# jianwen-xie/Latent-Space-Normalizing-Flow

Measured on AMD Instinct MI355X. Metric: latent-samples/sec through flow+logdet, nz=128 B=65536, higher is better.
Workload: dtype bf16x3; 1 GPU; CIFAR-10 flow prior nz=128 f_width=64 f_depth=5 affine, forward+logdet+log-prob, B=65536 synthetic z per evaluation (BASELINE.json configs[2]); rows_per_gpu=65536, global_rows=65536, parallelism=single GPU, streams=3, clock_ramp_launches_before_warmup=600

## Files before the change

### latent-space-normalizing-flow_amd/csrc/lsnf_device.h

```cpp
#pragma once
#include <hip/hip_runtime.h>
#include <type_traits>
#include "lsnf_layout.h"

typedef float f32x16 __attribute__((ext_vector_type(16)));
typedef float f32x4 __attribute__((ext_vector_type(4)));

#define LSNF_WG_THREADS 256
#define LSNF_WG_WAVES 4
#define LSNF_WG_SAMPLES (LSNF_WG_WAVES * 32)

#define LSNF_AS1 __attribute__((address_space(1)))
#define LSNF_AS3 __attribute__((address_space(3)))

static inline hipError_t lsnf_allow_big_lds(const void* kernel, unsigned long long* done_mask) {
    int dev = 0;
    hipError_t e = hipGetDevice(&dev);
    if (e != hipSuccess) return e;
    if (dev >= 0 && dev < 64 && ((*done_mask >> dev) & 1ull)) return hipSuccess;
    e = hipFuncSetAttribute(kernel, hipFuncAttributeMaxDynamicSharedMemorySize, 160 * 1024);
    if (e != hipSuccess) return e;
    if (dev >= 0 && dev < 64) *done_mask |= 1ull << dev;
    return hipSuccess;
}

template <template <int, int> class Cfg, class F>
static inline auto lsnf_with_cfg(const LsnfGeo& g, F&& f) {
    if (g.HT == 1) return f(Cfg<1, 1>{});
    if (g.WT == 2) return f(Cfg<2, 2>{});
    return f(Cfg<2, 4>{});
}

static inline unsigned long long* lsnf_stamps_buffer() {
#ifdef LSNF_STAMPS
    extern unsigned long long* g_lsnf_stamps;
    if (!g_lsnf_stamps && hipMalloc(&g_lsnf_stamps, sizeof(unsigned long long) * 64 * 4 * 4096) != hipSuccess) g_lsnf_stamps = nullptr;
    return g_lsnf_stamps;
#else
    return nullptr;
#endif
}

template <int HT_, int WT_>
struct LsnfStackCfg {
    static constexpr int HT = HT_, WT = WT_, NZT = 2 * HT_;
    static constexpr int P1 = NZT, P2 = WT, P3 = WT, P4 = 2 * HT, NP = P1 + P2 + P3 + P4;
    static constexpr int KT1 = NZT, KT2 = HT, KT3 = WT, KT4 = WT;
    static constexpr int OFF_S2 = LSNF_FRAG_FLOATS * P1 * KT1;
    static constexpr int OFF_S3 = OFF_S2 + LSNF_FRAG_FLOATS * P2 * KT2;
    static constexpr int OFF_S4 = OFF_S3 + LSNF_FRAG_FLOATS * P3 * KT3;
    static constexpr int FWD_BLOCK = OFF_S4 + LSNF_FRAG_FLOATS * P4 * KT4;
    static constexpr int FWD_CONST = 32 * NP + 32;
    static constexpr int INV_BLOCK = LSNF_FRAG_FLOATS * NZT * NZT;
    static constexpr int INV_CONST = 32 * NZT;
    static constexpr int OFF_B4 = 0;
    static constexpr int OFF_B3 = OFF_B4 + LSNF_FRAG_FLOATS * WT * 2 * HT;
    static constexpr int OFF_B2 = OFF_B3 + LSNF_FRAG_FLOATS * WT * WT;
    static constexpr int OFF_B1 = OFF_B2 + LSNF_FRAG_FLOATS * HT * WT;
    static constexpr int BWD_BLOCK = OFF_B1 + LSNF_FRAG_FLOATS * NZT * NZT;
    static constexpr int MAXKT = (NZT > WT ? NZT : WT);
    static constexpr int SLOT = 2 * MAXKT * LSNF_FRAG_FLOATS;
};

#define LSNF_STATS_SLOTS 64
__device__ __forceinline__ void lsnf_publish_stats(double* stats, double sum_ll, double sum_logdet, int rows, int lane) {
    const unsigned grid = gridDim.x, wg = blockIdx.x;
    unsigned long long* ticket = reinterpret_cast<unsigned long long*>(&stats[2]);
    int last = 0;
    if (lane == 0) {
        const unsigned s = wg % LSNF_STATS_SLOTS;
        double* sub = stats + 8 + 4 * s;
        const double r0 = atomicAdd(&sub[0], sum_ll);
        const double r1 = atomicAdd(&sub[1], sum_logdet);
        unsigned long long inc = 1ull;
        asm volatile("" : "+v"(inc) : "v"(r0), "v"(r1));
        bool slot_done = true;
        if (grid > LSNF_STATS_SLOTS) {
            const unsigned long long n_s = (grid - s + LSNF_STATS_SLOTS - 1) / LSNF_STATS_SLOTS;
            unsigned long long* st = reinterpret_cast<unsigned long long*>(&sub[2]);
            slot_done = atomicAdd(st, inc) == n_s - 1;
            if (slot_done) atomicExch(st, 0ull);
            inc = 1ull;
        }
        if (slot_done) {
            const unsigned long long slots = grid > LSNF_STATS_SLOTS ? LSNF_STATS_SLOTS : grid;
            if (atomicAdd(ticket, inc) == slots - 1) { last = 1; atomicExch(ticket, 0ull); }
        }
    }
    if (__builtin_amdgcn_readfirstlane(last)) {
        unsigned long long* sub = reinterpret_cast<unsigned long long*>(stats + 8 + 4 * lane);
        double fl = __longlong_as_double((long long)atomicExch(&sub[0], 0ull));
        double fd = __longlong_as_double((long long)atomicExch(&sub[1], 0ull));
#pragma unroll
        for (int o = 32; o > 0; o >>= 1) { fl += __shfl_xor(fl, o, 64); fd += __shfl_xor(fd, o, 64); }
        if (lane == 0) { stats[4] = fl; stats[5] = fd; stats[6] = (double)rows; }
    }
}

__device__ __forceinline__ constexpr int lsnf_feat(int r, int h) { return (r & 3) + 8 * (r >> 2) + 4 * h; }

template <int KT, int NW = LSNF_WG_WAVES>
__device__ __forceinline__ void lsnf_issue_panel(const float* __restrict__ gsrc, float* lbuf, int wave, int lane) {
#ifdef LSNF_ABLATE_DMA
    return;
#endif
    constexpr int PIECES = 4 * KT;
    constexpr int PER_WAVE = (PIECES + NW - 1) / NW;
#pragma unroll
    for (int s = 0; s < PER_WAVE; ++s) {
        const int seg = s * NW + wave;
        if (PIECES % NW == 0 || seg < PIECES) {
            const float* g = gsrc + seg * 256 + lane * 4;
            float* l = lbuf + seg * 256;
            __builtin_amdgcn_global_load_lds((const LSNF_AS1 void*)g, (LSNF_AS3 void*)l, 16, 0, 0);
        }
    }
}

__device__ __forceinline__ void lsnf_panel_barrier() {
    asm volatile("s_waitcnt vmcnt(0)" ::: "memory");
#ifndef LSNF_ABLATE_BARRIER
    __syncthreads();
#endif
}

template <int KT>
__device__ __forceinline__ void lsnf_panel_mma(f32x16& acc, const f32x16* in, const float* lbuf, int lane) {
    const f32x4* wp = reinterpret_cast<const f32x4*>(lbuf) + lane;
    __builtin_amdgcn_sched_barrier(0);
    f32x4 w0 = wp[0], w1 = wp[64], w2 = wp[128], w3 = wp[192];
    __builtin_amdgcn_sched_group_barrier(0x100, 4, 0);
#pragma unroll
    for (int kt = 0; kt < KT; ++kt) {
        f32x4 n0 = w0, n1 = w1, n2 = w2, n3 = w3;
        if (kt + 1 < KT) {
            n0 = wp[((kt + 1) * 4 + 0) * 64]; n1 = wp[((kt + 1) * 4 + 1) * 64];
            n2 = wp[((kt + 1) * 4 + 2) * 64]; n3 = wp[((kt + 1) * 4 + 3) * 64];
        }
#define LSNF_MFMA4(W, G)                                                                      \
        acc = __builtin_amdgcn_mfma_f32_32x32x2f32(W[0], in[kt][4 * G + 0], acc, 0, 0, 0);    \
        acc = __builtin_amdgcn_mfma_f32_32x32x2f32(W[1], in[kt][4 * G + 1], acc, 0, 0, 0);    \
        acc = __builtin_amdgcn_mfma_f32_32x32x2f32(W[2], in[kt][4 * G + 2], acc, 0, 0, 0);    \
        acc = __builtin_amdgcn_mfma_f32_32x32x2f32(W[3], in[kt][4 * G + 3], acc, 0, 0, 0);
        LSNF_MFMA4(w0, 0) LSNF_MFMA4(w1, 1) LSNF_MFMA4(w2, 2) LSNF_MFMA4(w3, 3)
#undef LSNF_MFMA4
        if (kt + 1 < KT) __builtin_amdgcn_sched_group_barrier(0x100, 4, 0);
        __builtin_amdgcn_sched_group_barrier(0x008, 16, 0);
        w0 = n0; w1 = n1; w2 = n2; w3 = n3;
    }
}

__device__ __forceinline__ f32x16 lsnf_bias_init(const float* cst, int h) {
    const f32x4* b = reinterpret_cast<const f32x4*>(cst + h * 16);
    f32x16 a;
#pragma unroll
    for (int q = 0; q < 4; ++q) {
        const f32x4 v = b[q];
        a[4 * q + 0] = v[0]; a[4 * q + 1] = v[1]; a[4 * q + 2] = v[2]; a[4 * q + 3] = v[3];
    }
    return a;
}

__device__ __forceinline__ f32x16 lsnf_zero16() {
    f32x16 a;
#pragma unroll
    for (int r = 0; r < 16; ++r) a[r] = 0.0f;
    return a;
}

__device__ __forceinline__ f32x16 lsnf_relu16(f32x16 a) {
#pragma unroll
    for (int r = 0; r < 16; ++r) a[r] = fmaxf(a[r], 0.0f);
    return a;
}

__device__ __forceinline__ void lsnf_sigmoid_log2(float p, float& sig, float& l2) {
    const float pc = __builtin_amdgcn_fmed3f(p, -80.0f, 80.0f);
    const float e = __builtin_amdgcn_exp2f(pc * -1.4426950408889634f);
    const float d = 1.0f + e;
    sig = __builtin_amdgcn_rcpf(d);
    l2 = __builtin_amdgcn_logf(d);
}

__device__ __forceinline__ void lsnf_sigmoid_logsig(float p, float& sig, float& lsig) {
#ifdef LSNF_ABLATE_EPILOGUE
    sig = p * 0.25f + 0.5f; lsig = p; return;
#endif
#ifdef LSNF_OCML_MATH
    const float a = fabsf(p);
    const float e = expf(-a);
    const float r = 1.0f / (1.0f + e);
    const float l = log1pf(e);
    sig = (p >= 0.0f) ? r : e * r;
    lsig = fminf(p, 0.0f) - l;
#else
    float l2;
    lsnf_sigmoid_log2(p, sig, l2);
    lsig = -0.6931471805599453f * l2;
#endif
}

__device__ __forceinline__ float lsnf_pair_add16(float v) {
    const unsigned u = __builtin_bit_cast(unsigned, v);
    const auto r = __builtin_amdgcn_permlane16_swap(u, u, false, false);
    return __builtin_bit_cast(float, (unsigned)r[0]) + __builtin_bit_cast(float, (unsigned)r[1]);
}
__device__ __forceinline__ float lsnf_pair_add32(float v) {
    const unsigned u = __builtin_bit_cast(unsigned, v);
    const auto r = __builtin_amdgcn_permlane32_swap(u, u, false, false);
    return __builtin_bit_cast(float, (unsigned)r[0]) + __builtin_bit_cast(float, (unsigned)r[1]);
}
__device__ __forceinline__ unsigned lsnf_pair_or32(unsigned u) {
    const auto r = __builtin_amdgcn_permlane32_swap(u, u, false, false);
    return (unsigned)r[0] | (unsigned)r[1];
}
__device__ __forceinline__ float lsnf_pair_sum(float v) { return lsnf_pair_add32(v); }

typedef float f32x2 __attribute__((ext_vector_type(2)));
template <int HT>
__device__ __forceinline__ f32x16 lsnf_load_tile(int t, const float* __restrict__ zr, int half, int h, int vw) {
    f32x16 x;
    const int hh = t / HT, tt = t % HT;
#pragma unroll
    for (int g = 0; g < 4; ++g) {
        const int f0 = 32 * tt + 8 * g + 4 * h;
        const int col0 = hh * half + f0;
        if (vw == 4) {
            f32x4 v = {0.f, 0.f, 0.f, 0.f};
            if (f0 < half) v = *reinterpret_cast<const f32x4*>(zr + col0);
            x[4 * g + 0] = v[0]; x[4 * g + 1] = v[1]; x[4 * g + 2] = v[2]; x[4 * g + 3] = v[3];
        } else if (vw == 2) {
            f32x2 v0 = {0.f, 0.f}, v1 = {0.f, 0.f};
            if (f0 < half) v0 = *reinterpret_cast<const f32x2*>(zr + col0);
            if (f0 + 2 < half) v1 = *reinterpret_cast<const f32x2*>(zr + col0 + 2);
            x[4 * g + 0] = v0[0]; x[4 * g + 1] = v0[1]; x[4 * g + 2] = v1[0]; x[4 * g + 3] = v1[1];
        } else {
#pragma unroll
            for (int j = 0; j < 4; ++j) x[4 * g + j] = (f0 + j < half) ? zr[col0 + j] : 0.0f;
        }
    }
    return x;
}

template <int HT>
__device__ __forceinline__ void lsnf_store_tile(int t, const f32x16& x, float* __restrict__ zr, int half, int h, int vw) {
    const int hh = t / HT, tt = t % HT;
#pragma unroll
    for (int g = 0; g < 4; ++g) {
        const int f0 = 32 * tt + 8 * g + 4 * h;
// ... 189 lines not shown
```

### latent-space-normalizing-flow_amd/csrc/lsnf_fwd3p.hip

```cpp
#include <stdlib.h>
#include <type_traits>
#include "lsnf_l16.h"

#if LSNF_L16_PARTS != 3
#error "lsnf_fwd3p.hip is the three-term bf16 kernel"
#endif

#ifndef LSNF_FILLMASK
#define LSNF_FILLMASK 0x7f
#endif

namespace {

struct Fwd3pArgs {
    const float* consts; const float* panels3;
    const float* z_in; const float* objective;
    float* z_out; float* logdet_out; float* ll_out;
    int B, nz, half, n_blocks, vec4;
    double* stats;
    float* hdump; int width;
    float* z_saved; float* act_saved;
    unsigned long long* stamps;
};

// ... 118 lines not shown
    for (int r = r0; r < r0 + 2 * ST; ++r) {
        float sig, l2;
        lsnf_sigmoid_log2(p.q[qr][r], sig, l2);
        p.q[qr][r] = sig; lsum[st] += l2;
    }
    keep(p.q[qr][r0], p.q[qr][r0 + 1], p.q[qr][r0 + 2 * ST - 2], p.q[qr][r0 + 2 * ST - 1], lsum[st]);
}
template <int ST>
__device__ __forceinline__ void couple_q16(Tile16& v, const Tile16& t, const Tile16& sig, int q) {
    const int qr = unit_quad<ST>(q), r0 = 2 * unit_pair0<ST>(q);
#pragma unroll
    for (int r = r0; r < r0 + 2 * ST; ++r) v.q[qr][r] = (v.q[qr][r] + t.q[qr][r]) * sig.q[qr][r];
}

#ifndef LSNF_STASH_AUX
#define LSNF_STASH_AUX 0
#endif
#ifndef LSNF_STASH_PARTS
#define LSNF_STASH_PARTS 7
#endif
typedef unsigned u32x4s __attribute__((ext_vector_type(4)));
struct StashLane { unsigned zoff, soff, moff, msh, hoff; };
struct StashRsrc { __amdgpu_buffer_rsrc_t r[2]; };
__device__ __forceinline__ StashRsrc stash_rsrc(const float* p, unsigned bytes, unsigned second_off) {
    char* c = reinterpret_cast<char*>(const_cast<float*>(p));
    return StashRsrc{{__builtin_amdgcn_make_buffer_rsrc(c, 0, (int)bytes, 0x00020000),
                      __builtin_amdgcn_make_buffer_rsrc(c + second_off, 0, (int)(bytes > second_off ? bytes - second_off : 0u), 0x00020000)}};
}
template <int HT>
__device__ __forceinline__ void stash_row_quad(const StashRsrc& rs, const StashLane& sl, int t, int q, const Tile16& x, int nz, int half, int g) {
    if constexpr (!(LSNF_STASH_PARTS & 4)) return;
    const int ft = q >> 1, st = q & 1, hh = t / HT, tt = t % HT;
    unsigned off = sl.zoff;
    if (st) off += (unsigned)(16 * nz * 4);
    off = (32 * tt + 16 * ft + 4 * g < half) ? off : 0x80000000u;
    const u32x4s v = __builtin_bit_cast(u32x4s, x.q[q]);
    __builtin_amdgcn_raw_buffer_store_b128(v, rs.r[hh], off + (unsigned)((32 * tt + 16 * ft) * 4), 0, LSNF_STASH_AUX);
}
__device__ __forceinline__ void stash_sigma_quad(const StashRsrc& rs, const StashLane& sl, int t, int q, const Tile16& sg) {
    if constexpr (!(LSNF_STASH_PARTS & 2)) return;
    const int ft = q >> 1, st = q & 1;
    const u32x4s v = __builtin_bit_cast(u32x4s, sg.q[q]);
    __builtin_amdgcn_raw_buffer_store_b128(v, rs.r[t], sl.soff + (unsigned)((2 * ft * 64 + 16 * st) * 16), 0, LSNF_STASH_AUX);
}
__device__ __forceinline__ void mask_q16(const Tile16& h, int q, unsigned (&mk)[2][2]) {
    if constexpr (!(LSNF_STASH_PARTS & 1)) return;
    unsigned m = 0;
#pragma unroll
    for (int r = 3; r >= 0; --r) m = __builtin_amdgcn_alignbit(m, __builtin_bit_cast(unsigned, 0.0f - h.q[q][r]), 31);
    mk[q & 1][q >> 1] = m;
    asm volatile("" :: "v"(m));
}
__device__ __forceinline__ void stash_mask_words(const StashRsrc& rs, const StashLane& sl, int tile, const unsigned (&mk)[2][2]) {
    if constexpr (!(LSNF_STASH_PARTS & 1)) return;
    const unsigned w0 = mk[0][0] | (mk[0][1] << 8), w1 = mk[1][0] | (mk[1][1] << 8);
    unsigned x = ((w0 << 16) | w1) << sl.msh;
    x = lsnf_pair_or32(x);
    __builtin_amdgcn_raw_buffer_store_b32(x >> 16, rs.r[0], sl.moff + (unsigned)(tile * 64 * 4), 0, 0);
    __builtin_amdgcn_raw_buffer_store_b32(x & 0xffffu, rs.r[0], sl.moff + (unsigned)((tile * 64 + 16) * 4), 0, 0);
}
__device__ __forceinline__ void stash_h_quad(const StashRsrc& rs, const StashLane& sl, int t, int q, const Tile16& h, int width) {
    const int ft = q >> 1, st = q & 1;
    f32x4v r;
#pragma unroll
    for (int j = 0; j < 4; ++j) r[j] = fmaxf(h.q[q][j], 0.0f);
    const unsigned off = (32 * t + 16 * ft < width) ? sl.hoff : 0x80000000u;
    __builtin_amdgcn_raw_buffer_store_b128(__builtin_bit_cast(u32x4s, r), rs.r[t], off + (unsigned)((ft * 2 + st) * 1024), 0, LSNF_STASH_AUX);
}

template <int NM, int NV>
__device__ __forceinline__ void pin_mfma() {
    lsnf_static_for<NM>([&](auto mc) {
        constexpr int m = decltype(mc)::value, V = NV / NM + (m < NV % NM ? 1 : 0);
        __builtin_amdgcn_sched_group_barrier(0x008, 1, 0);
        if constexpr (V > 0) __builtin_amdgcn_sched_group_barrier(0x402, V, 0);
    });
}
template <class PH, int ST, class Fill, class Mid>
__device__ __forceinline__ void run_phase16(Tile16* acc, const float* bias_ptr , const SplitTile16* in, const float* lbuf, int lane, Fill&& fill, Mid&& mid) {
    const bf16x8* wp = reinterpret_cast<const bf16x8*>(lbuf) + lane;
    __builtin_amdgcn_sched_barrier(0);
    bf16x8 a[3];
#pragma unroll
    for (int p = 0; p < 3; ++p) a[p] = wp[(PH::at(0).frag + p) * 64];
    f32x4v bq = bias_quad(bias_ptr, 32 * PH::btile(PH::at(0).acc) + 8 * PH::at(0).s);
    __builtin_amdgcn_sched_group_barrier(0x100, 4, 0);
    lsnf_static_for<PH::N>([&](auto ic) {
        constexpr int i = decltype(ic)::value;
        constexpr StepDesc d = PH::at(i);
        mid(ic);
        bf16x8 na[3];
        f32x4v nbq = bq;
#pragma unroll
        for (int p = 0; p < 3; ++p) na[p] = a[p];
        if constexpr (i + 1 < PH::N) {
#pragma unroll
            for (int p = 0; p < 3; ++p) na[p] = wp[(PH::at(i + 1).frag + p) * 64];
            if constexpr (first_touch<PH>(i + 1)) nbq = bias_quad(bias_ptr, 32 * PH::btile(PH::at(i + 1).acc) + 8 * PH::at(i + 1).s);
        }
#ifndef LSNF_ABL_NOFILL
        fill(ic);
#endif
        const SplitTile16& x = in[d.tile];
        constexpr bool first = first_touch<PH>(i);
#define LSNF_Q_MMA(WI, XI) \
        acc[d.acc].q[2 * d.s + 0] = __builtin_amdgcn_mfma_f32_16x16x32_bf16(a[WI], __builtin_bit_cast(bf16x8, u32x4{x.d[0][XI][0], x.d[0][XI][1], x.d[0][XI][2], x.d[0][XI][3]}), (first && WI == 2 && XI == 0) ? bq : acc[d.acc].q[2 * d.s + 0], 0, 0, 0); \
        if constexpr (ST == 2) acc[d.acc].q[2 * d.s + 1] = __builtin_amdgcn_mfma_f32_16x16x32_bf16(a[WI], __builtin_bit_cast(bf16x8, u32x4{x.d[1][XI][0], x.d[1][XI][1], x.d[1][XI][2], x.d[1][XI][3]}), (first && WI == 2 && XI == 0) ? bq : acc[d.acc].q[2 * d.s + 1], 0, 0, 0);
#ifdef LSNF_ABL_NOMFMA
        LSNF_Q_MMA(0, 0)
#else
        LSNF_F3_TERMS(LSNF_Q_MMA)
#endif
#undef LSNF_Q_MMA
        if constexpr (i + 1 < PH::N) __builtin_amdgcn_sched_group_barrier(0x100, first_touch<PH>(i + 1) ? 4 : 3, 0);
        pin_mfma<6 * ST, (PH::valu(i) * ST) / 2>();
        __builtin_amdgcn_sched_barrier(0);
#pragma unroll
        for (int p = 0; p < 3; ++p) a[p] = na[p];
        bq = nbq;
    });
}

struct QhNoStores { static constexpr int stores(int) { return 0; } };
struct QhS1a : QhNoStores {
    static constexpr int N = 16;
    static constexpr int btile(int acc) { return acc; }
    static constexpr StepDesc at(int i) { return mkstep<4>((i >> 1) & 1, (i >> 1) & 1, i >> 2, i >> 2, i & 1); }
    static constexpr int valu(int i) { return i < 2 ? 22 : (i < 6 ? 28 : (i < 8 ? 16 : (i < 12 ? 22 : 0))); }
};
struct QhS1b : QhNoStores {
    static constexpr int N = 16;
    static constexpr int btile(int acc) { return 2 + acc; }
    static constexpr StepDesc at(int i) { return mkstep<4>((i >> 1) & 1, (i >> 1) & 1, i >> 2, i >> 2, i & 1); }
    static constexpr int valu(int i) { return i >= 8 ? 22 : 0; }
};
struct QhS23 : QhNoStores {
    static constexpr int N = 16;
    static constexpr int btile(int acc) { return 4 + acc; }
    static constexpr StepDesc at(int i) {
        if (i < 8) { const int tl = i >> 2, kt = (i >> 1) & 1; return mkstep<2>(tl, tl, kt, kt, i & 1); }
        const int j = i - 8, kt = j >> 2, tl = (j >> 1) & 1;
        return mkstep<2>(2 + tl, 2 + tl, 2 + kt, kt, j & 1);
    }
    static constexpr int valu(int i) { return (i >= 4 && i < 12) ? 26 : (i >= 13 ? 26 : 0); }
};
struct QhS4 : QhNoStores {
    static constexpr int N = 16;
    static constexpr int btile(int acc) { return 8 + (acc == 0 ? 2 : (acc == 1 ? 0 : (acc == 2 ? 3 : 1))); }
    static constexpr int torder(int j) { return j == 0 ? 2 : (j == 1 ? 0 : (j == 2 ? 3 : 1)); }
    static constexpr StepDesc at(int i) { const int kt = i >> 3, j = (i >> 1) & 3; return mkstep<2>(j, torder(j), kt, kt, i & 1); }
    static constexpr int valu(int i) { return i < 4 ? 26 : (i < 9 ? 0 : (i < 12 ? 28 : (i == 12 ? 36 : (i == 13 ? 24 : 22)))); }
};

struct QsS1a : QhS1a {
    static constexpr int valu(int i) { return (i == 6 || i == 7) ? 20 : (i >= 8 && i < 12 ? 23 : QhS1a::valu(i)); }
    static constexpr int stores(int i) { return (i >= 2 && i < 6) ? 1 : ((i == 6 || i == 7) ? 2 : (i >= 8 && i < 12 ? 1 : 0)); }
};
struct QsS1b : QhS1b {
    static constexpr int valu(int i) { return i < 8 ? (i >= 6 ? 1 : 0) : (i < 14 ? 23 : 22); }
    static constexpr int stores(int i) { return (i >= 6 && i < 14) ? 1 : 0; }
};
struct QsS23 : QhS23 {
    static constexpr int valu(int i) { return (i >= 4 && i < 12) ? (i == 8 ? 44 : 34) : (i >= 13 ? 34 : 0); }
    static constexpr int stores(int i) { return i == 8 ? 2 : 0; }
};
struct QsS4 : QhS4 {
    static constexpr int valu(int i) { return i < 4 ? 34 : ((i >= 6 && i < 9) ? 10 + QhS4::valu(i) : QhS4::valu(i)); }
    static constexpr int stores(int i) { return (i >= 6 && i < 9) ? 2 : ((i >= 9 && i < 13) ? 1 : 0); }
};
struct QxS23 : QsS23 {
    static constexpr int valu(int i) { return QsS23::valu(i) + (((i >= 4 && i < 12) || i >= 13) ? 2 : 0); }
    static constexpr int stores(int i) { return QsS23::stores(i) + (((i >= 4 && i < 12) || i >= 13) ? 1 : 0); }
};
struct QxS4 : QsS4 {
    static constexpr int valu(int i) { return QsS4::valu(i) + (i < 4 ? 2 : 0); }
    static constexpr int stores(int i) { return QsS4::stores(i) + (i < 4 ? 1 : 0); }
};
template <class PH> constexpr int stores_after(int last_dma_step) {
    int n = 0;
    for (int i = last_dma_step + 1; i < PH::N; ++i) n += PH::stores(i);
    return n;
}

template <int WT, int NWAVES, int ST, int STASH = 0>
__global__ __launch_bounds__(64 * NWAVES, 1) void lsnf_fwd3q_kernel(const Fwd3pArgs a) {
    static_assert(!STASH || ST == 2, "the stash tile is a wave's 32 rows");
    using TS1a = std::conditional_t<STASH != 0, QsS1a, QhS1a>;
    using TS1b = std::conditional_t<STASH != 0, QsS1b, QhS1b>;
    using TS23 = std::conditional_t<STASH == 2, QxS23, std::conditional_t<STASH != 0, QsS23, QhS23>>;
    using TS4 = std::conditional_t<STASH == 2, QxS4, std::conditional_t<STASH != 0, QsS4, QhS4>>;
    using C = Fwd3pCfg<WT>;
    static_assert(WT == 2, "lsnf_fwd3q_kernel: f_width <= 64 instantiation");
    constexpr int THREADS = 64 * NWAVES;
    constexpr int HT = 2, NZT = 4, F = C::F;
    constexpr int SLOT = C::SLOT3;
    extern __shared__ __attribute__((aligned(16))) float smem[];
    float* cst = smem;
    float* const buf0 = smem + a.n_blocks * C::CONST_FLOATS;
    const int tid = threadIdx.x;
    const int wave = __builtin_amdgcn_readfirstlane(tid >> 6);
    const int lane = tid & 63;
    const int n = lane & 15, g = lane >> 4;
    P_STAMP(0, "s_memtime");
    P_STAMP(50, "s_memrealtime");
    const int n_phases = 4 * a.n_blocks;
    auto phase_src = [&](int k) -> const float* {
        const float* gb = a.panels3 + (size_t)(k >> 2) * C::BLOCK3;
        const int j = k & 3;
        return gb + (j == 0 ? 0 : (j == 1 ? 2 * 4 * F : (j == 2 ? C::OFF3_S2 : C::OFF3_S4)));
    };
    auto sync_issue = [&](int k, auto left) {
#ifdef LSNF_ABL_SKIPSYNC
        if ((LSNF_ABL_SKIPSYNC >> (k & 3)) & 1) return;
#endif
        asm volatile("s_waitcnt vmcnt(%0)" :: "n"(decltype(left)::value) : "memory");
        __syncthreads();
#ifdef LSNF_FWD3Q_BURST_DMA
        if (k + 1 < n_phases) issue_kib<48, NWAVES>(phase_src(k + 1), buf0 + ((k + 1) & 1) * SLOT, wave, lane);
#endif
    };
    constexpr int PER_WAVE = 48 / NWAVES, EVERY = STASH ? 1 : 16 / PER_WAVE, LAST_DMA = (PER_WAVE - 1) * EVERY;
    using Left0 = std::integral_constant<int, 0>;
    using LeftS1a = std::integral_constant<int, stores_after<TS1a>(LAST_DMA)>;
    using LeftS1b = std::integral_constant<int, stores_after<TS1b>(LAST_DMA)>;
    using LeftS23 = std::integral_constant<int, stores_after<TS23>(LAST_DMA) + (STASH == 2 ? 1 : 0)>;
    using LeftS4 = std::integral_constant<int, stores_after<TS4>(LAST_DMA)>;
    const float* dma_src = nullptr; float* dma_dst = nullptr;
    auto dma_arm = [&](int k) {
        dma_src = phase_src(k + 1 < n_phases ? k + 1 : k);
        dma_dst = buf0 + ((k + 1) & 1) * SLOT;
    };
    auto dma_step = [&](auto ic) {
#ifndef LSNF_FWD3Q_BURST_DMA
        constexpr int i = decltype(ic)::value;
        if constexpr (i % EVERY == 0 && i / EVERY < PER_WAVE) issue_piece<NWAVES>(dma_src, dma_dst, i / EVERY, wave, lane);
#endif
    };

    const int wbase = (blockIdx.x * NWAVES + wave) * (16 * ST);
    int sample[2] = {0, 0}, rows[2] = {0, 0}; bool live[2] = {false, false};
#pragma unroll
    for (int st = 0; st < ST; ++st) { sample[st] = wbase + 16 * st + n; live[st] = sample[st] < a.B; rows[st] = live[st] ? sample[st] : a.B - 1; }

    Tile16 v[NZT];
    SplitTile16 xs[NZT];
    Tile16 p1, t1;
    float lsum[2] = {0.0f, 0.0f};
    {
        const Tile16 x0 = load_tile16<HT, ST>(0, a.z_in, rows, a.nz, a.half, g, a.vec4);
        const Tile16 x1 = load_tile16<HT, ST>(1, a.z_in, rows, a.nz, a.half, g, a.vec4);
        v[2] = load_tile16<HT, ST>(2, a.z_in, rows, a.nz, a.half, g, a.vec4);
        v[3] = load_tile16<HT, ST>(3, a.z_in, rows, a.nz, a.half, g, a.vec4);
        __builtin_amdgcn_sched_barrier(0);
        issue_kib<48, NWAVES>(phase_src(0), buf0, wave, lane);
        for (int i = tid; i < a.n_blocks * C::CONST_FLOATS; i += THREADS) cst[i] = a.consts[i];
#pragma unroll
        for (int q = 0; q < 4; ++q) { split_q16<false, ST>(x0, q, xs[0]); split_q16<false, ST>(x1, q, xs[1]); }
        split_q16<false, ST>(v[2], 0, xs[2]); split_q16<false, ST>(v[2], 1, xs[2]);
#pragma unroll
        for (int q = 0; q < 4; ++q)
#pragma unroll
            for (int r = 0; r < 4; ++r) { p1.q[q][r] = 80.0f; t1.q[q][r] = 0.0f; }
    }
    float ell[2];
#pragma unroll
    for (int st = 0; st < 2; ++st) ell[st] = (st < ST && a.objective) ? a.objective[rows[st]] : 0.0f;
    float ss01[2] = {0.0f, 0.0f};
    StashLane sl0 = {0u, 0u, 0u, 0u};
    const LsnfActLayout al = lsnf_act_layout(a.B, HT, WT);
    const unsigned zbytes = (unsigned)a.B * (unsigned)a.nz * 4u, abytes = (unsigned)(al.per_block * 4);
    if constexpr (STASH) {
        const unsigned tile_byte = (unsigned)(wbase >> 5) * (unsigned)(al.per_tile * 4), L = (unsigned)(n + 32 * (g & 1));
        sl0.zoff = ((unsigned)(wbase + n) * (unsigned)a.nz + 4u * g) * 4u;
        sl0.soff = tile_byte + ((unsigned)(g >> 1) * 64u + L) * 16u;
        sl0.moff = tile_byte + (unsigned)(al.mask_off * 4) + L * 4u;
        sl0.msh = 4u * (g >> 1);
        sl0.hoff = (unsigned)(wbase >> 5) * (unsigned)(32 * a.width * 4) + (unsigned)(n * 4 + g) * 16u;
    }
    const LsnfDumpLayout dl = lsnf_dump_layout(a.B, a.nz, a.width);
    const unsigned hbytes = (unsigned)(((size_t)a.B + 31) / 32 * 32 * a.width * 4);
    sync_issue(0, Left0{});
    P_STAMP(1, "s_memtime");

    for (int blk = 0; blk < a.n_blocks; ++blk) {
        const float* cb = cst + blk * C::CONST_FLOATS;
        const bool more = blk + 1 < a.n_blocks;
        const int k0 = 4 * blk;
        SplitTile16 vh[4];
        SplitTile16 h2s[WT];
        Tile16 hh[4], tp[4];
        const bool zs = STASH && a.z_saved != nullptr, as = STASH && a.act_saved != nullptr;
        const float* zc = more ? (zs ? a.z_saved + (size_t)blk * a.B * a.nz : a.z_out) : a.z_out;
        const float* zp = blk > 0 ? (zs ? a.z_saved + (size_t)(blk - 1) * a.B * a.nz : a.z_out) : a.z_out;
        const StashRsrc rs_zc = stash_rsrc(zc, (more && !zs) ? 0u : zbytes, (unsigned)a.half * 4u);
        const StashRsrc rs_zp = stash_rsrc(zp, (blk > 0 && !zs) ? 0u : zbytes, (unsigned)a.half * 4u);
        const StashRsrc rs_ac = stash_rsrc(as ? a.act_saved + (size_t)blk * al.per_block : a.z_out, as ? abytes : 0u, 4096u);
        const StashRsrc rs_ap = stash_rsrc(as ? a.act_saved + (size_t)(blk > 0 ? blk - 1 : 0) * al.per_block : a.z_out, as ? abytes : 0u, 4096u);
        StashLane sl = sl0;
        if constexpr (STASH) asm volatile("" : "+v"(sl.zoff), "+v"(sl.soff), "+v"(sl.moff));
        if constexpr (STASH == 2) asm volatile("" : "+v"(sl.hoff));
        const float* hd = (STASH == 2) ? a.hdump + (size_t)blk * dl.per_block : a.z_out;
        const StashRsrc rs_h1 = stash_rsrc(STASH == 2 ? hd + dl.off_h1 : hd, STASH == 2 ? hbytes : 0u, 4096u);
        const StashRsrc rs_h2 = stash_rsrc(STASH == 2 ? hd + dl.off_h2 : hd, STASH == 2 ? hbytes : 0u, 4096u);
        unsigned mk1[2][2], mk2[2][2], mk3[2][2];

        if (blk == 1) P_STAMP(10, "s_memtime");
        {
            const float* bv = bias_lane_ptr(cb, g);
            if (k0 > 0) sync_issue(k0, LeftS4{});
            dma_arm(k0);
            run_phase16<TS1a, ST>(v, bv, xs, buf0 + (k0 & 1) * SLOT, lane, [&](auto ic) {
                constexpr int i = decltype(ic)::value;
                if constexpr (STASH && i >= 8 && i < 12) stash_row_quad<HT>(rs_zp, sl, 2, i - 8, v[2], a.nz, a.half, g);
                if constexpr (i < 2) split_q16<false, ST>(v[2], 2 + i, xs[2]);
                else if constexpr (i < 6) {
                    sigmoid_q16<ST>(p1, i - 2, lsum);
                    if constexpr (STASH) stash_sigma_quad(rs_ap, sl, 1, i - 2, p1);
                } else if constexpr (i < 8) {
                    couple_q16<ST>(v[3], t1, p1, 2 * (i - 6)); couple_q16<ST>(v[3], t1, p1, 2 * (i - 6) + 1);
                    if constexpr (STASH) { stash_row_quad<HT>(rs_zp, sl, 3, 2 * (i - 6), v[3], a.nz, a.half, g); stash_row_quad<HT>(rs_zp, sl, 3, 2 * (i - 6) + 1, v[3], a.nz, a.half, g); }
                } else if constexpr (i < 12) split_q16<false, ST>(v[3], i - 8, xs[3]);
            }, dma_step);
        }
        if (blk == 1) P_STAMP(11, "s_memtime");
        {
            const float* bv = bias_lane_ptr(cb, g);
            sync_issue(k0 + 1, LeftS1a{});
            dma_arm(k0 + 1);
            run_phase16<TS1b, ST>(v + 2, bv, xs, buf0 + ((k0 + 1) & 1) * SLOT, lane, [&](auto ic) {
                constexpr int i = decltype(ic)::value;
                if constexpr (STASH && i >= 6 && i < 14) stash_row_quad<HT>(rs_zc, sl, (i - 6) >> 2, (i - 6) & 3, v[(i - 6) >> 2], a.nz, a.half, g);
                if constexpr (i >= 8) split_q16<false, ST>(v[(i - 8) >> 2], i & 3, vh[(i - 8) >> 2]);
            }, dma_step);
        }
        if (blk == 1) P_STAMP(12, "s_memtime");
        if (!more) {
            int ln = lane;
            asm volatile("" : "+v"(ln));
            const int smp[2] = {wbase + (ln & 15), wbase + 16 + (ln & 15)};
#pragma unroll
            for (int t = 0; t < HT; ++t) {
                if constexpr (!STASH) store_tile16<HT, ST>(t, v[t], a.z_out, smp, live, a.nz, a.half, g, a.vec4);
#pragma unroll
                for (int ft = 0; ft < 2; ++ft)
#pragma unroll
                    for (int st = 0; st < ST; ++st)
#pragma unroll
                        for (int r = 0; r < 4; ++r) ss01[st] += v[t].q[2 * ft + st][r] * v[t].q[2 * ft + st][r];
            }
        }
#pragma unroll
        for (int st = 0; st < 2; ++st) { ell[st] = ell[st] + cb[32 * C::NP + 0]; ell[st] = ell[st] + cb[32 * C::NP + 1]; }
        {
            static_assert(C::P1 == 4 && C::P2 == 2 && C::P3 == 2, "bias tile indices of the phase tables");
            const float* bv = bias_lane_ptr(cb, g);
            sync_issue(k0 + 2, LeftS1b{});
            dma_arm(k0 + 2);
            run_phase16<TS23, ST>(hh, bv, vh, buf0 + ((k0 + 2) & 1) * SLOT, lane, [&](auto ic) {
                constexpr int i = decltype(ic)::value;
                if constexpr (i >= 4 && i < 8) split_q16<true, ST>(hh[0], i - 4, vh[2]);
                if constexpr (i >= 8 && i < 12) split_q16<true, ST>(hh[1], i - 8, vh[3]);
                if constexpr (i >= 13) split_q16<true, ST>(hh[2], i - 13, h2s[0]);
                if constexpr (STASH) {
                    if constexpr (i >= 4 && i < 8) mask_q16(hh[0], i - 4, mk3);
                    if constexpr (i == 8) stash_mask_words(rs_ac, sl, 0, mk3);
                    if constexpr (i >= 8 && i < 12) mask_q16(hh[1], i - 8, mk1);
                    if constexpr (i >= 13) mask_q16(hh[2], i - 13, mk2);
                }
                if constexpr (STASH == 2) {
                    if constexpr (i >= 4 && i < 8) stash_h_quad(rs_h1, sl, 0, i - 4, hh[0], a.width);
                    if constexpr (i >= 8 && i < 12) stash_h_quad(rs_h1, sl, 1, i - 8, hh[1], a.width);
                    if constexpr (i >= 13) stash_h_quad(rs_h2, sl, 0, i - 13, hh[2], a.width);
                }
            }, dma_step);
        }
        if (blk == 1) P_STAMP(13, "s_memtime");
        xs[0] = vh[0]; xs[1] = vh[1];
        {
            constexpr int B4 = C::P1 + C::P2 + C::P3;
            static_assert(B4 == 8, "bias tile indices of the phase tables");
            const float* bv = bias_lane_ptr(cb, g);
            split_q16<true, ST>(hh[2], 3, h2s[0]);
            if constexpr (STASH) mask_q16(hh[2], 3, mk2);
            if constexpr (STASH == 2) stash_h_quad(rs_h2, sl, 0, 3, hh[2], a.width);
            sync_issue(k0 + 3, LeftS23{});
            dma_arm(k0 + 3);
            run_phase16<TS4, ST>(tp, bv, h2s, buf0 + ((k0 + 3) & 1) * SLOT, lane, [&](auto ic) {
                constexpr int i = decltype(ic)::value;
                if constexpr (i < 4) split_q16<true, ST>(hh[3], i, h2s[1]);
                if constexpr (STASH) {
                    if constexpr (i < 4) mask_q16(hh[3], i, mk3);
                    if constexpr (i == 6) stash_mask_words(rs_ac, sl, 1, mk1);
                    if constexpr (i == 7) stash_mask_words(rs_ac, sl, WT + 0, mk2);
                    if constexpr (i == 8) stash_mask_words(rs_ac, sl, WT + 1, mk3);
                }
                if constexpr (STASH == 2 && i < 4) stash_h_quad(rs_h2, sl, 1, i, hh[3], a.width);
                if constexpr (i >= 9 && i < 13) { sigmoid_q16<ST>(tp[0], i - 9, lsum); if constexpr (STASH) stash_sigma_quad(rs_ac, sl, 0, i - 9, tp[0]); }
                if constexpr (i == 12) couple_q16<ST>(v[2], tp[1], tp[0], 0);
                if constexpr (i == 13) { couple_q16<ST>(v[2], tp[1], tp[0], 1); couple_q16<ST>(v[2], tp[1], tp[0], 2); couple_q16<ST>(v[2], tp[1], tp[0], 3); }
                if constexpr (i >= 14) split_q16<false, ST>(v[2], i - 14, xs[2]);
            }, dma_step);
            p1 = tp[2]; t1 = tp[3];
        }
        if (blk == 1) P_STAMP(14, "s_memtime");
    }
    P_STAMP(40, "s_memtime");
#pragma unroll
    for (int q = 0; q < 4; ++q) { sigmoid_q16<ST>(p1, q, lsum); couple_q16<ST>(v[3], t1, p1, q); }
    if constexpr (STASH) {
        const bool as = a.act_saved != nullptr;
        const StashRsrc rs_al = stash_rsrc(as ? a.act_saved + (size_t)(a.n_blocks - 1) * al.per_block : a.z_out, as ? abytes : 0u, 4096u);
#pragma unroll
        for (int q = 0; q < 4; ++q) stash_sigma_quad(rs_al, sl0, 1, q, p1);
    }
#pragma unroll
    for (int st = 0; st < ST; ++st) ell[st] = ell[st] + -0.6931471805599453f * l16_group_sum(lsum[st]);

    float ss[2] = {ss01[0], ss01[1]};
    int ln_e = lane;
    asm volatile("" : "+v"(ln_e));
    const int smp_e[2] = {wbase + (ln_e & 15), wbase + 16 + (ln_e & 15)};
#pragma unroll
    for (int t = HT; t < NZT; ++t) {
#pragma unroll
        for (int ft = 0; ft < 2; ++ft)
#pragma unroll
            for (int st = 0; st < ST; ++st)
#pragma unroll
                for (int r = 0; r < 4; ++r) ss[st] += v[t].q[2 * ft + st][r] * v[t].q[2 * ft + st][r];
        store_tile16<HT, ST>(t, v[t], a.z_out, smp_e, live, a.nz, a.half, g, a.vec4);
    }
    float ll[2] = {0.0f, 0.0f};
#pragma unroll
    for (int st = 0; st < ST; ++st) {
        ll[st] = (-0.5f * l16_group_sum(ss[st]) + 1.8378770664093453f) + ell[st];
        if (live[st] && g == 0) {
            const int smp = smp_e[st];
            a.logdet_out[smp] = ell[st];
            if (a.ll_out) a.ll_out[smp] = ll[st];
        }
    }
    asm volatile("s_waitcnt vmcnt(0)" ::: "memory");
    if (a.stats) {
        double dl = 0.0, dd = 0.0;
#pragma unroll
        for (int st = 0; st < ST; ++st)
            if (live[st] && g == 0) { dl += (double)ll[st]; dd += (double)ell[st]; }
#pragma unroll
        for (int o = 8; o > 0; o >>= 1) { dl += __shfl_xor(dl, o, 64); dd += __shfl_xor(dd, o, 64); }
        __syncthreads();
        double* red = reinterpret_cast<double*>(buf0);
        if (lane == 0) { red[2 * wave] = dl; red[2 * wave + 1] = dd; }
        __syncthreads();
        if (wave == 0) {
            double tl = 0.0, td = 0.0;
            for (int w = 0; w < NWAVES; ++w) { tl += red[2 * w]; td += red[2 * w + 1]; }
            lsnf_publish_stats(a.stats, tl, td, a.B, lane);
        }
    }
    P_STAMP(41, "s_memtime");
    P_STAMP(51, "s_memrealtime");
}

size_t fwd3q_lds(int n_blocks) {
    using C = Fwd3pCfg<2>;
    return ((size_t)n_blocks * C::CONST_FLOATS + 2 * (size_t)C::SLOT3) * sizeof(float);
}

template <int WT, int NWAVES, int ST, int STASH = 0>
hipError_t launch_fwd3q_w(const Fwd3pArgs& a, hipStream_t stream) {
    const size_t lds = fwd3q_lds(a.n_blocks);
    auto kern = lsnf_fwd3q_kernel<WT, NWAVES, ST, STASH>;
    static unsigned long long lds_ok = 0;
    if (hipError_t e = lsnf_allow_big_lds((const void*)kern, &lds_ok); e != hipSuccess) return e;
    const unsigned grid = (unsigned)((a.B + 16 * ST * NWAVES - 1) / (16 * ST * NWAVES));
    hipLaunchKernelGGL(kern, dim3(grid), dim3(64 * NWAVES), lds, stream, a);
    return hipGetLastError();
}
}

bool lsnf_forward3q_covers(const LsnfGeo& g, int first_block, int n_blocks, int B, int vec4, const float* z_out,
                           const float* z_saved, const float* act_saved, const float* hdump, int hdump_tiled) {
    if (g.HT != 2 || g.WT != 2 || fwd3q_lds(n_blocks) > 160 * 1024) return false;
    if (hdump && (!hdump_tiled || !act_saved || (n_blocks > 1 && !z_saved) || first_block != 0 || (g.width & 15) ||
                  ((size_t)B + 32) * g.width * 4 >= (1ull << 31))) return false;
    const bool stash = act_saved != nullptr || z_saved != nullptr;
    return !(stash && (vec4 != 4 || (size_t)B * g.nz * 4 >= (1ull << 31) || lsnf_act_layout(B, g.HT, g.WT).per_block * 4 >= (1ull << 31) ||
                       (((size_t)act_saved | (size_t)z_saved | (size_t)z_out) & 15)));
}

hipError_t lsnf_launch_forward3q(const LsnfGeo& g, const float* plan, int first_block, int n_blocks, int B,
                                 const float* z_in, const float* objective, float* z_out, float* logdet_out,
                                 float* ll_out, float* z_saved, float* act_saved, double* stats, int vec4, hipStream_t stream,
                                 float* hdump, int hdump_tiled) {
    if (!lsnf_forward3q_covers(g, first_block, n_blocks, B, vec4, z_out, z_saved, act_saved, hdump, hdump_tiled))
        return hipErrorInvalidValue;
    const bool stash = act_saved != nullptr || z_saved != nullptr;
    Fwd3pArgs a;
    a.consts = plan + g.off_fwd_const + (size_t)first_block * g.fwd_const_floats;
    a.panels3 = plan + g.off_f3b_panels + (size_t)first_block * g.f3_block_floats;
    a.z_in = z_in; a.objective = objective; a.z_out = z_out; a.logdet_out = logdet_out; a.ll_out = ll_out;
    a.B = B; a.nz = g.nz; a.half = g.half; a.n_blocks = n_blocks; a.vec4 = vec4; a.stats = stats;
    a.z_saved = z_saved; a.act_saved = act_saved ? act_saved + (size_t)first_block * lsnf_act_layout(B, g.HT, g.WT).per_block : nullptr;
    a.hdump = hdump; a.width = g.width;
    a.stamps = lsnf_stamps_buffer();
    static const char* shape = getenv("LSNF_FWD3Q_SHAPE");
    const int sh = shape ? atoi(shape) : (B > 128 * 256 ? 82 : (B > 64 * 256 ? 81 : 41));
    if (hdump) return (sh == 82) ? launch_fwd3q_w<2, 8, 2, 2>(a, stream) : launch_fwd3q_w<2, 4, 2, 2>(a, stream);
    if (stash) return (sh == 82) ? launch_fwd3q_w<2, 8, 2, 1>(a, stream) : launch_fwd3q_w<2, 4, 2, 1>(a, stream);
    if (sh == 82) return launch_fwd3q_w<2, 8, 2>(a, stream);
    if (sh == 42) return launch_fwd3q_w<2, 4, 2>(a, stream);
    if (sh == 81) return launch_fwd3q_w<2, 8, 1>(a, stream);
    return launch_fwd3q_w<2, 4, 1>(a, stream);
}
```

Baseline: 756.9 million latent-samples/s.

## Restructure fwd3q prologue/epilogue to overlap input loads, constants copy and final stores

Result: slower. 745.5 million latent-samples/s (-1.5%).

```diff
diff --git a/latent-space-normalizing-flow_amd/csrc/lsnf_device.h b/latent-space-normalizing-flow_amd/csrc/lsnf_device.h
--- a/latent-space-normalizing-flow_amd/csrc/lsnf_device.h
+++ b/latent-space-normalizing-flow_amd/csrc/lsnf_device.h
@@ -63,17 +63,25 @@
 };
 
 #define LSNF_STATS_SLOTS 64
-__device__ __forceinline__ void lsnf_publish_stats(double* stats, double sum_ll, double sum_logdet, int rows, int lane) {
+struct LsnfStatsAdds { double r0, r1; };
+__device__ __forceinline__ LsnfStatsAdds lsnf_publish_stats_issue(double* stats, double sum_ll, double sum_logdet, int lane) {
+    LsnfStatsAdds p = {0.0, 0.0};
+    if (lane == 0) {
+        double* sub = stats + 8 + 4 * (blockIdx.x % LSNF_STATS_SLOTS);
+        p.r0 = atomicAdd(&sub[0], sum_ll);
+        p.r1 = atomicAdd(&sub[1], sum_logdet);
+    }
+    return p;
+}
+__device__ __forceinline__ void lsnf_publish_stats_finish(double* stats, const LsnfStatsAdds& p, int rows, int lane) {
     const unsigned grid = gridDim.x, wg = blockIdx.x;
     unsigned long long* ticket = reinterpret_cast<unsigned long long*>(&stats[2]);
     int last = 0;
     if (lane == 0) {
         const unsigned s = wg % LSNF_STATS_SLOTS;
         double* sub = stats + 8 + 4 * s;
-        const double r0 = atomicAdd(&sub[0], sum_ll);
-        const double r1 = atomicAdd(&sub[1], sum_logdet);
         unsigned long long inc = 1ull;
-        asm volatile("" : "+v"(inc) : "v"(r0), "v"(r1));
+        asm volatile("" : "+v"(inc) : "v"(p.r0), "v"(p.r1));
         bool slot_done = true;
         if (grid > LSNF_STATS_SLOTS) {
             const unsigned long long n_s = (grid - s + LSNF_STATS_SLOTS - 1) / LSNF_STATS_SLOTS;
@@ -95,6 +103,9 @@
         for (int o = 32; o > 0; o >>= 1) { fl += __shfl_xor(fl, o, 64); fd += __shfl_xor(fd, o, 64); }
         if (lane == 0) { stats[4] = fl; stats[5] = fd; stats[6] = (double)rows; }
     }
+}
+__device__ __forceinline__ void lsnf_publish_stats(double* stats, double sum_ll, double sum_logdet, int rows, int lane) {
+    lsnf_publish_stats_finish(stats, lsnf_publish_stats_issue(stats, sum_ll, sum_logdet, lane), rows, lane);
 }
 
 __device__ __forceinline__ constexpr int lsnf_feat(int r, int h) { return (r & 3) + 8 * (r >> 2) + 4 * h; }
diff --git a/latent-space-normalizing-flow_amd/csrc/lsnf_fwd3p.hip b/latent-space-normalizing-flow_amd/csrc/lsnf_fwd3p.hip
--- a/latent-space-normalizing-flow_amd/csrc/lsnf_fwd3p.hip
+++ b/latent-space-normalizing-flow_amd/csrc/lsnf_fwd3p.hip
@@ -294,6 +294,10 @@
     static constexpr int valu(int i) { return i < 4 ? 26 : (i < 9 ? 0 : (i < 12 ? 28 : (i == 12 ? 36 : (i == 13 ? 24 : 22)))); }
 };
 
+struct QhS1aFirst : QhS1a {
+    static constexpr int valu(int i) { return (i < 12 && (i & 3) >= 2) ? 44 : 0; }
+};
+
 struct QsS1a : QhS1a {
     static constexpr int valu(int i) { return (i == 6 || i == 7) ? 20 : (i >= 8 && i < 12 ? 23 : QhS1a::valu(i)); }
     static constexpr int stores(int i) { return (i >= 2 && i < 6) ? 1 : ((i == 6 || i == 7) ? 2 : (i >= 8 && i < 12 ? 1 : 0)); }
@@ -318,6 +322,22 @@
     static constexpr int valu(int i) { return QsS4::valu(i) + (i < 4 ? 2 : 0); }
     static constexpr int stores(int i) { return QsS4::stores(i) + (i < 4 ? 1 : 0); }
 };
+template <int HT, int ST>
+__device__ __forceinline__ Tile16 load_tile16_buf(int t, const StashRsrc& rs, unsigned zoff, int nz, int half, int g) {
+    Tile16 x;
+    const int hh = t / HT, tt = t % HT;
+#pragma unroll
+    for (int ft = 0; ft < 2; ++ft)
+#pragma unroll
+        for (int st = 0; st < ST; ++st) {
+            unsigned off = zoff + (unsigned)(st * 16 * nz * 4);
+            off = (32 * tt + 16 * ft + 4 * g < half) ? off : 0x80000000u;
+            const u32x4s v = __builtin_amdgcn_raw_buffer_load_b128(rs.r[hh], off + (unsigned)((32 * tt + 16 * ft) * 4), 0, 0);
+            x.q[2 * ft + st] = __builtin_bit_cast(f32x4v, v);
+        }
+    return x;
+}
+
 template <class PH> constexpr int stores_after(int last_dma_step) {
     int n = 0;
     for (int i = last_dma_step + 1; i < PH::N; ++i) n += PH::stores(i);
@@ -328,6 +348,7 @@
 __global__ __launch_bounds__(64 * NWAVES, 1) void lsnf_fwd3q_kernel(const Fwd3pArgs a) {
     static_assert(!STASH || ST == 2, "the stash tile is a wave's 32 rows");
     using TS1a = std::conditional_t<STASH != 0, QsS1a, QhS1a>;
+    using TS1aF = QhS1aFirst;
     using TS1b = std::conditional_t<STASH != 0, QsS1b, QhS1b>;
     using TS23 = std::conditional_t<STASH == 2, QxS23, std::conditional_t<STASH != 0, QsS23, QhS23>>;
     using TS4 = std::conditional_t<STASH == 2, QxS4, std::conditional_t<STASH != 0, QsS4, QhS4>>;
@@ -355,7 +376,7 @@
 #ifdef LSNF_ABL_SKIPSYNC
         if ((LSNF_ABL_SKIPSYNC >> (k & 3)) & 1) return;
 #endif
-        asm volatile("s_waitcnt vmcnt(%0)" :: "n"(decltype(left)::value) : "memory");
+        if constexpr (decltype(left)::value >= 0) asm volatile("s_waitcnt vmcnt(%0)" :: "n"(decltype(left)::value) : "memory");
         __syncthreads();
 #ifdef LSNF_FWD3Q_BURST_DMA
         if (k + 1 < n_phases) issue_kib<48, NWAVES>(phase_src(k + 1), buf0 + ((k + 1) & 1) * SLOT, wave, lane);
@@ -363,6 +384,7 @@
     };
     constexpr int PER_WAVE = 48 / NWAVES, EVERY = STASH ? 1 : 16 / PER_WAVE, LAST_DMA = (PER_WAVE - 1) * EVERY;
     using Left0 = std::integral_constant<int, 0>;
+    using LeftWaited = std::integral_constant<int, -1>;
     using LeftS1a = std::integral_constant<int, stores_after<TS1a>(LAST_DMA)>;
     using LeftS1b = std::integral_constant<int, stores_after<TS1b>(LAST_DMA)>;
     using LeftS23 = std::integral_constant<int, stores_after<TS23>(LAST_DMA) + (STASH == 2 ? 1 : 0)>;
@@ -389,20 +411,45 @@
     Tile16 p1, t1;
     float lsum[2] = {0.0f, 0.0f};
     {
-        const Tile16 x0 = load_tile16<HT, ST>(0, a.z_in, rows, a.nz, a.half, g, a.vec4);
-        const Tile16 x1 = load_tile16<HT, ST>(1, a.z_in, rows, a.nz, a.half, g, a.vec4);
-        v[2] = load_tile16<HT, ST>(2, a.z_in, rows, a.nz, a.half, g, a.vec4);
-        v[3] = load_tile16<HT, ST>(3, a.z_in, rows, a.nz, a.half, g, a.vec4);
+        const bool rows16 = a.vec4 == 4;
+        const unsigned wg_row0 = blockIdx.x * (unsigned)(NWAVES * 16 * ST);
+        const unsigned wg_rows = min((unsigned)a.B - wg_row0, (unsigned)(NWAVES * 16 * ST));
+        const StashRsrc rs_in = stash_rsrc(a.z_in + (size_t)wg_row0 * a.nz, rows16 ? wg_rows * (unsigned)a.nz * 4u : 0u, (unsigned)a.half * 4u);
+        const unsigned zoff_in = ((unsigned)(wave * 16 * ST + n) * (unsigned)a.nz + 4u * g) * 4u;
+        Tile16 x0;
+        if (rows16) x0 = load_tile16_buf<HT, ST>(0, rs_in, zoff_in, a.nz, a.half, g);
+        else x0 = load_tile16<HT, ST>(0, a.z_in, rows, a.nz, a.half, g, a.vec4);
         __builtin_amdgcn_sched_barrier(0);
         issue_kib<48, NWAVES>(phase_src(0), buf0, wave, lane);
-        for (int i = tid; i < a.n_blocks * C::CONST_FLOATS; i += THREADS) cst[i] = a.consts[i];
-#pragma unroll
-        for (int q = 0; q < 4; ++q) { split_q16<false, ST>(x0, q, xs[0]); split_q16<false, ST>(x1, q, xs[1]); }
-        split_q16<false, ST>(v[2], 0, xs[2]); split_q16<false, ST>(v[2], 1, xs[2]);
-#pragma unroll
-        for (int q = 0; q < 4; ++q)
-#pragma unroll
-            for (int r = 0; r < 4; ++r) { p1.q[q][r] = 80.0f; t1.q[q][r] = 0.0f; }
+        {
+            constexpr int U = 32 / NWAVES;
+            const int total4 = a.n_blocks * (C::CONST_FLOATS / 4);
+            static_assert(C::CONST_FLOATS % 4 == 0, "constant blocks are copied in 16-byte groups");
+            const f32x4* src4 = reinterpret_cast<const f32x4*>(a.consts);
+            f32x4* dst4 = reinterpret_cast<f32x4*>(cst);
+            for (int base = 0; base < total4; base += U * THREADS) {
+                f32x4 c[U];
+#pragma unroll
+                for (int u = 0; u < U; ++u) { const int i = base + u * THREADS + tid; c[u] = src4[i < total4 ? i : total4 - 1]; }
+#pragma unroll
+                for (int u = 0; u < U; ++u) { const int i = base + u * THREADS + tid; if (i < total4) dst4[i] = c[u]; }
+            }
+        }
+        __builtin_amdgcn_s_waitcnt(0x0f70);
+        __builtin_amdgcn_sched_barrier(0);
+        if (rows16) {
+            p1 = load_tile16_buf<HT, ST>(1, rs_in, zoff_in, a.nz, a.half, g);
+            v[2] = load_tile16_buf<HT, ST>(2, rs_in, zoff_in, a.nz, a.half, g);
+            v[3] = load_tile16_buf<HT, ST>(3, rs_in, zoff_in, a.nz, a.half, g);
+        } else {
+            p1 = load_tile16<HT, ST>(1, a.z_in, rows, a.nz, a.half, g, a.vec4);
+            v[2] = load_tile16<HT, ST>(2, a.z_in, rows, a.nz, a.half, g, a.vec4);
+            v[3] = load_tile16<HT, ST>(3, a.z_in, rows, a.nz, a.half, g, a.vec4);
+            __builtin_amdgcn_s_waitcnt(0x0f70);
+        }
+        __builtin_amdgcn_sched_barrier(0);
+#pragma unroll
+        for (int q = 0; q < 4; ++q) split_q16<false, ST>(x0, q, xs[0]);
     }
     float ell[2];
 #pragma unroll
@@ -421,10 +468,20 @@
     }
     const LsnfDumpLayout dl = lsnf_dump_layout(a.B, a.nz, a.width);
     const unsigned hbytes = (unsigned)(((size_t)a.B + 31) / 32 * 32 * a.width * 4);
-    sync_issue(0, Left0{});
+    sync_issue(0, LeftWaited{});
     P_STAMP(1, "s_memtime");
-
-    for (int blk = 0; blk < a.n_blocks; ++blk) {
+    dma_arm(0);
+    run_phase16<TS1aF, ST>(v, bias_lane_ptr(cst, g), xs, buf0, lane, [&](auto ic) {
+        constexpr int i = decltype(ic)::value;
+        if constexpr (i < 12 && (i & 3) >= 2) {
+            constexpr int q = 2 * ((i & 3) - 2);
+            const Tile16& x = (i >> 2) == 0 ? p1 : v[1 + (i >> 2)];
+            split_q16<false, ST>(x, q, xs[1 + (i >> 2)]); split_q16<false, ST>(x, q + 1, xs[1 + (i >> 2)]);
+        }
+    }, dma_step);
+    P_STAMP(2, "s_memtime");
+
+    for (int blk = 0;; ++blk) {
         const float* cb = cst + blk * C::CONST_FLOATS;
         const bool more = blk + 1 < a.n_blocks;
         const int k0 = 4 * blk;
@@ -433,11 +490,8 @@
         Tile16 hh[4], tp[4];
         const bool zs = STASH && a.z_saved != nullptr, as = STASH && a.act_saved != nullptr;
         const float* zc = more ? (zs ? a.z_saved + (size_t)blk * a.B * a.nz : a.z_out) : a.z_out;
-        const float* zp = blk > 0 ? (zs ? a.z_saved + (size_t)(blk - 1) * a.B * a.nz : a.z_out) : a.z_out;
         const StashRsrc rs_zc = stash_rsrc(zc, (more && !zs) ? 0u : zbytes, (unsigned)a.half * 4u);
-        const StashRsrc rs_zp = stash_rsrc(zp, (blk > 0 && !zs) ? 0u : zbytes, (unsigned)a.half * 4u);
         const StashRsrc rs_ac = stash_rsrc(as ? a.act_saved + (size_t)blk * al.per_block : a.z_out, as ? abytes : 0u, 4096u);
-        const StashRsrc rs_ap = stash_rsrc(as ? a.act_saved + (size_t)(blk > 0 ? blk - 1 : 0) * al.per_block : a.z_out, as ? abytes : 0u, 4096u);
         StashLane sl = sl0;
         if constexpr (STASH) asm volatile("" : "+v"(sl.zoff), "+v"(sl.soff), "+v"(sl.moff));
         if constexpr (STASH == 2) asm volatile("" : "+v"(sl.hoff));
@@ -446,28 +500,10 @@
         const StashRsrc rs_h2 = stash_rsrc(STASH == 2 ? hd + dl.off_h2 : hd, STASH == 2 ? hbytes : 0u, 4096u);
         unsigned mk1[2][2], mk2[2][2], mk3[2][2];
 
-        if (blk == 1) P_STAMP(10, "s_memtime");
         {
             const float* bv = bias_lane_ptr(cb, g);
-            if (k0 > 0) sync_issue(k0, LeftS4{});
-            dma_arm(k0);
-            run_phase16<TS1a, ST>(v, bv, xs, buf0 + (k0 & 1) * SLOT, lane, [&](auto ic) {
-                constexpr int i = decltype(ic)::value;
-                if constexpr (STASH && i >= 8 && i < 12) stash_row_quad<HT>(rs_zp, sl, 2, i - 8, v[2], a.nz, a.half, g);
-                if constexpr (i < 2) split_q16<false, ST>(v[2], 2 + i, xs[2]);
-                else if constexpr (i < 6) {
-                    sigmoid_q16<ST>(p1, i - 2, lsum);
-                    if constexpr (STASH) stash_sigma_quad(rs_ap, sl, 1, i - 2, p1);
-                } else if constexpr (i < 8) {
-                    couple_q16<ST>(v[3], t1, p1, 2 * (i - 6)); couple_q16<ST>(v[3], t1, p1, 2 * (i - 6) + 1);
-                    if constexpr (STASH) { stash_row_quad<HT>(rs_zp, sl, 3, 2 * (i - 6), v[3], a.nz, a.half, g); stash_row_quad<HT>(rs_zp, sl, 3, 2 * (i - 6) + 1, v[3], a.nz, a.half, g); }
-                } else if constexpr (i < 12) split_q16<false, ST>(v[3], i - 8, xs[3]);
-            }, dma_step);
-        }
-        if (blk == 1) P_STAMP(11, "s_memtime");
-        {
-            const float* bv = bias_lane_ptr(cb, g);
-            sync_issue(k0 + 1, LeftS1a{});
+            if (STASH && blk == 0) sync_issue(k0 + 1, Left0{});
+            else sync_issue(k0 + 1, LeftS1a{});
             dma_arm(k0 + 1);
             run_phase16<TS1b, ST>(v + 2, bv, xs, buf0 + ((k0 + 1) & 1) * SLOT, lane, [&](auto ic) {
                 constexpr int i = decltype(ic)::value;
@@ -545,44 +581,68 @@
             p1 = tp[2]; t1 = tp[3];
         }
         if (blk == 1) P_STAMP(14, "s_memtime");
+        if (!more) break;
+        if (blk == 0) P_STAMP(10, "s_memtime");
+        {
+            const float* bv = bias_lane_ptr(cb + C::CONST_FLOATS, g);
+            sync_issue(k0 + 4, LeftS4{});
+            dma_arm(k0 + 4);
+            run_phase16<TS1a, ST>(v, bv, xs, buf0 + (k0 & 1) * SLOT, lane, [&](auto ic) {
+                constexpr int i = decltype(ic)::value;
+                if constexpr (STASH && i >= 8 && i < 12) stash_row_quad<HT>(rs_zc, sl, 2, i - 8, v[2], a.nz, a.half, g);
+                if constexpr (i < 2) split_q16<false, ST>(v[2], 2 + i, xs[2]);
+                else if constexpr (i < 6) {
+                    sigmoid_q16<ST>(p1, i - 2, lsum);
+                    if constexpr (STASH) stash_sigma_quad(rs_ac, sl, 1, i - 2, p1);
+                } else if constexpr (i < 8) {
+                    couple_q16<ST>(v[3], t1, p1, 2 * (i - 6)); couple_q16<ST>(v[3], t1, p1, 2 * (i - 6) + 1);
+                    if constexpr (STASH) { stash_row_quad<HT>(rs_zc, sl, 3, 2 * (i - 6), v[3], a.nz, a.half, g); stash_row_quad<HT>(rs_zc, sl, 3, 2 * (i - 6) + 1, v[3], a.nz, a.half, g); }
+                } else if constexpr (i < 12) split_q16<false, ST>(v[3], i - 8, xs[3]);
+            }, dma_step);
+        }
+        if (blk == 0) P_STAMP(11, "s_memtime");
     }
     P_STAMP(40, "s_memtime");
 #pragma unroll
     for (int q = 0; q < 4; ++q) { sigmoid_q16<ST>(p1, q, lsum); couple_q16<ST>(v[3], t1, p1, q); }
+#pragma unroll
+    for (int st = 0; st < ST; ++st) ell[st] = ell[st] + -0.6931471805599453f * l16_group_sum(lsum[st]);
+
+    float ss[2] = {ss01[0], ss01[1]};
+#pragma unroll
+    for (int t = HT; t < NZT; ++t)
+#pragma unroll
+        for (int ft = 0; ft < 2; ++ft)
+#pragma unroll
+            for (int st = 0; st < ST; ++st)
+#pragma unroll
+                for (int r = 0; r < 4; ++r) ss[st] += v[t].q[2 * ft + st][r] * v[t].q[2 * ft + st][r];
+    float ll[2] = {0.0f, 0.0f};
+#pragma unroll
+    for (int st = 0; st < ST; ++st) ll[st] = (-0.5f * l16_group_sum(ss[st]) + 1.8378770664093453f) + ell[st];
+    int ln_e = lane;
+    asm volatile("" : "+v"(ln_e));
+    const int smp_e[2] = {wbase + (ln_e & 15), wbase + 16 + (ln_e & 15)};
+    auto final_stores = [&]() {
+#pragma unroll
+        for (int t = HT; t < NZT; ++t) store_tile16<HT, ST>(t, v[t], a.z_out, smp_e, live, a.nz, a.half, g, a.vec4);
+#pragma unroll
+        for (int st = 0; st < ST; ++st)
+            if (live[st] && g == 0) {
+                const int smp = smp_e[st];
+                a.logdet_out[smp] = ell[st];
+                if (a.ll_out) a.ll_out[smp] = ll[st];
+            }
+    };
+    asm volatile("s_waitcnt vmcnt(%0)" :: "n"(LeftS4::value) : "memory");
+    __builtin_amdgcn_sched_barrier(0);
+    P_STAMP(42, "s_memtime");
     if constexpr (STASH) {
         const bool as = a.act_saved != nullptr;
         const StashRsrc rs_al = stash_rsrc(as ? a.act_saved + (size_t)(a.n_blocks - 1) * al.per_block : a.z_out, as ? abytes : 0u, 4096u);
 #pragma unroll
         for (int q = 0; q < 4; ++q) stash_sigma_quad(rs_al, sl0, 1, q, p1);
     }
-#pragma unroll
-    for (int st = 0; st < ST; ++st) ell[st] = ell[st] + -0.6931471805599453f * l16_group_sum(lsum[st]);
-
-    float ss[2] = {ss01[0], ss01[1]};
-    int ln_e = lane;
-    asm volatile("" : "+v"(ln_e));
-    const int smp_e[2] = {wbase + (ln_e & 15), wbase + 16 + (ln_e & 15)};
-#pragma unroll
-    for (int t = HT; t < NZT; ++t) {
-#pragma unroll
-        for (int ft = 0; ft < 2; ++ft)
-#pragma unroll
-            for (int st = 0; st < ST; ++st)
-#pragma unroll
-                for (int r = 0; r < 4; ++r) ss[st] += v[t].q[2 * ft + st][r] * v[t].q[2 * ft + st][r];
-        store_tile16<HT, ST>(t, v[t], a.z_out, smp_e, live, a.nz, a.half, g, a.vec4);
-    }
-    float ll[2] = {0.0f, 0.0f};
-#pragma unroll
-    for (int st = 0; st < ST; ++st) {
-        ll[st] = (-0.5f * l16_group_sum(ss[st]) + 1.8378770664093453f) + ell[st];
-        if (live[st] && g == 0) {
-            const int smp = smp_e[st];
-            a.logdet_out[smp] = ell[st];
-            if (a.ll_out) a.ll_out[smp] = ll[st];
-        }
-    }
-    asm volatile("s_waitcnt vmcnt(0)" ::: "memory");
     if (a.stats) {
         double dl = 0.0, dd = 0.0;
 #pragma unroll
@@ -590,15 +650,26 @@
             if (live[st] && g == 0) { dl += (double)ll[st]; dd += (double)ell[st]; }
 #pragma unroll
         for (int o = 8; o > 0; o >>= 1) { dl += __shfl_xor(dl, o, 64); dd += __shfl_xor(dd, o, 64); }
-        __syncthreads();
-        double* red = reinterpret_cast<double*>(buf0);
+        double* red = reinterpret_cast<double*>(buf0 + 2 * SLOT);
         if (lane == 0) { red[2 * wave] = dl; red[2 * wave + 1] = dd; }
-        __syncthreads();
         if (wave == 0) {
+            __syncthreads();
             double tl = 0.0, td = 0.0;
             for (int w = 0; w < NWAVES; ++w) { tl += red[2 * w]; td += red[2 * w + 1]; }
-            lsnf_publish_stats(a.stats, tl, td, a.B, lane);
-        }
+            const LsnfStatsAdds pend = lsnf_publish_stats_issue(a.stats, tl, td, lane);
+            __builtin_amdgcn_sched_barrier(0);
+            final_stores();
+            __builtin_amdgcn_sched_barrier(0);
+            P_STAMP(43, "s_memtime");
+            lsnf_publish_stats_finish(a.stats, pend, a.B, lane);
+        } else {
+            final_stores();
+            P_STAMP(43, "s_memtime");
+            __syncthreads();
+        }
+    } else {
+        final_stores();
+        P_STAMP(43, "s_memtime");
     }
     P_STAMP(41, "s_memtime");
     P_STAMP(51, "s_memrealtime");
@@ -606,7 +677,7 @@
 
 size_t fwd3q_lds(int n_blocks) {
     using C = Fwd3pCfg<2>;
-    return ((size_t)n_blocks * C::CONST_FLOATS + 2 * (size_t)C::SLOT3) * sizeof(float);
+    return ((size_t)n_blocks * C::CONST_FLOATS + 2 * (size_t)C::SLOT3 + 32) * sizeof(float);
 }
 
 template <int WT, int NWAVES, int ST, int STASH = 0>
```
